# tjqansthd/GDN-Pytorch

Hardware: AMD Instinct MI355X
Metric: training images/sec at 128x416 batch=20 (higher is better)
Workload: dtype f32; 1 GPU; DtoD training step (fwd + losses + bwd + fused Adam), batch 20 per GPU, 128x416, fp32, BASELINE configs[1]; global_batch=20, parallelism=dp1, launch=eager, x3=True

## Files before the change

gdn-pytorch_amd/csrc/gemm_x3.hip:

```cpp
#include "gemm_x3.h"


namespace {

__global__ __launch_bounds__(256) void x3_pack_rows_kernel(const float* __restrict__ src, unsigned char* __restrict__ dst, int rows,
                                                           int K, int rows_pad) {
    const int KB = K / X3_BK, k8n = K / 8;
    const int bin = blockIdx.y;
    const size_t per_bin = x3_packed_bytes(rows, K);
    for (int64_t i = blockIdx.x * 256ll + threadIdx.x; i < (int64_t)rows_pad * k8n; i += (int64_t)gridDim.x * 256) {
        const int row = (int)((i >> 2) % rows_pad), k8 = (int)(i & 3) + 4 * (int)((i >> 2) / rows_pad);
        f32x4 lo = {0.f, 0.f, 0.f, 0.f}, hi = lo;
        if (row < rows) {
            const float* s = src + ((size_t)bin * rows + row) * K + k8 * 8;
            lo = *reinterpret_cast<const f32x4*>(s);
            hi = *reinterpret_cast<const f32x4*>(s + 4);
        }
        unsigned h[3][4];
        x3_split2(lo[0], lo[1], h[0][0], h[1][0], h[2][0]);
        x3_split2(lo[2], lo[3], h[0][1], h[1][1], h[2][1]);
        x3_split2(hi[0], hi[1], h[0][2], h[1][2], h[2][2]);
        x3_split2(hi[2], hi[3], h[0][3], h[1][3], h[2][3]);
#pragma unroll
        for (int p = 0; p < 3; ++p) {
            const uint4 v = {h[p][0], h[p][1], h[p][2], h[p][3]};
            *reinterpret_cast<uint4*>(dst + (size_t)bin * per_bin + x3_off(row, k8 * 8, p, KB)) = v;
        }
    }
}

__device__ __forceinline__ void x3_stage_mfma(const unsigned char* As, const unsigned char* Bs, int a_base, int b_base, int h, int f_sw,
                                              f32x16 (&acc)[2][2], f32x16 (&cor)[2][2]) {
#pragma unroll
    for (int s = 0; s < 2; ++s) {
        const int co = ((2 * s + h) ^ f_sw) * 16;
        x3_bf16x8 af[2][3], bf[2][3];
#pragma unroll
        for (int i = 0; i < 2; ++i)
#pragma unroll
            for (int p = 0; p < 3; ++p) {
                af[i][p] = __builtin_bit_cast(x3_bf16x8, *reinterpret_cast<const uint4*>(&As[p * 8192 + a_base + i * 2048 + co]));
                bf[i][p] = __builtin_bit_cast(x3_bf16x8, *reinterpret_cast<const uint4*>(&Bs[p * 8192 + b_base + i * 2048 + co]));
            }
#pragma unroll
        for (int i = 0; i < 2; ++i)
#pragma unroll
            for (int j = 0; j < 2; ++j) {
                cor[i][j] = __builtin_amdgcn_mfma_f32_32x32x16_bf16(af[i][2], bf[j][0], cor[i][j], 0, 0, 0);
                cor[i][j] = __builtin_amdgcn_mfma_f32_32x32x16_bf16(af[i][1], bf[j][1], cor[i][j], 0, 0, 0);
                cor[i][j] = __builtin_amdgcn_mfma_f32_32x32x16_bf16(af[i][0], bf[j][2], cor[i][j], 0, 0, 0);
                cor[i][j] = __builtin_amdgcn_mfma_f32_32x32x16_bf16(af[i][1], bf[j][0], cor[i][j], 0, 0, 0);
                cor[i][j] = __builtin_amdgcn_mfma_f32_32x32x16_bf16(af[i][0], bf[j][1], cor[i][j], 0, 0, 0);
                acc[i][j] = __builtin_amdgcn_mfma_f32_32x32x16_bf16(af[i][0], bf[j][0], acc[i][j], 0, 0, 0);
            }
    }
}

__global__ __launch_bounds__(256, 2) void gemm_x3_nt_kernel(const float* __restrict__ A, const unsigned char* __restrict__ Bp,
                                                            float* __restrict__ C, int M, int N, int K, int bins) {
    __shared__ __attribute__((aligned(16))) unsigned char As[3 * 128 * 64], Bs[3 * 128 * 64];
    const int tid = threadIdx.x, lane = tid & 63, wave = tid >> 6, wm = wave >> 1, wn = wave & 1;
    const int NT = N / 128, MT = (M + 127) / 128, KB = K / X3_BK;
    const int xcd = blockIdx.x & 7, sq = blockIdx.x >> 3;
    const int bin = (sq / (NT * MT)) * 8 + xcd;
    if (bin >= bins) return;
    const int m0 = ((sq / NT) % MT) * 128, nt = sq % NT;
    const float* Ab = A + (size_t)bin * M * K;
    const unsigned char* Bb = Bp + (size_t)bin * x3_packed_bytes(N, K) + (size_t)nt * KB * (3 * 128 * 64);
    float* Cb = C + (size_t)bin * M * N;

    f32x16 acc[2][2], cor[2][2];
#pragma unroll
    for (int i = 0; i < 2; ++i)
#pragma unroll
        for (int j = 0; j < 2; ++j)
#pragma unroll
            for (int r = 0; r < 16; ++r) { acc[i][j][r] = 0.f; cor[i][j][r] = 0.f; }

    const int k4 = tid & 7, rb0 = tid >> 3;
    const float* ap[4];
#pragma unroll
    for (int v = 0; v < 4; ++v) {
        const int row = v * 32 + rb0;
        ap[v] = Ab + (size_t)(m0 + row < M ? m0 + row : M - 1) * K + k4 * 4;
    }
    f32x4 ra[4];
    f32x4 rb[6];
    auto gload = [&](int kb) {
#pragma unroll
        for (int v = 0; v < 4; ++v) ra[v] = *reinterpret_cast<const f32x4*>(ap[v] + (size_t)kb * X3_BK);
        const unsigned char* bsrc = Bb + (size_t)kb * (3 * 128 * 64) + tid * 16;
#pragma unroll
        for (int v = 0; v < 6; ++v) rb[v] = *reinterpret_cast<const f32x4*>(bsrc + v * 4096);
    };
    auto lstore = [&]() {
#pragma unroll
        for (int v = 0; v < 4; ++v) {
            const int row = v * 32 + rb0;
            unsigned h0[3], h1[3];
            x3_split2(ra[v][0], ra[v][1], h0[0], h0[1], h0[2]);
            x3_split2(ra[v][2], ra[v][3], h1[0], h1[1], h1[2]);
            const int off = row * 64 + (((k4 >> 1) ^ x3_sw(row)) * 16) + (k4 & 1) * 8;
#pragma unroll
            for (int p = 0; p < 3; ++p) {
                const uint2 w = {h0[p], h1[p]};
                *reinterpret_cast<uint2*>(&As[p * 8192 + off]) = w;
            }
        }
#pragma unroll
        for (int v = 0; v < 6; ++v) *reinterpret_cast<f32x4*>(&Bs[v * 4096 + tid * 16]) = rb[v];
    };
    const int r32 = lane & 31, h = lane >> 5;
    const int f_sw = x3_sw(r32);
    const int a_base = (wm * 64 + r32) * 64, b_base = (wn * 64 + r32) * 64;

    gload(0);
    for (int kb = 0; kb < KB; ++kb) {
        lstore();
        __syncthreads();
        if (kb + 1 < KB) gload(kb + 1);
        x3_stage_mfma(As, Bs, a_base, b_base, h, f_sw, acc, cor);
        __syncthreads();
    }
#pragma unroll
    for (int i = 0; i < 2; ++i)
#pragma unroll
        for (int j = 0; j < 2; ++j) {
            const int col = nt * 128 + wn * 64 + j * 32 + r32;
#pragma unroll
            for (int r = 0; r < 16; ++r) {
                const int m = m0 + wm * 64 + i * 32 + (r & 3) + 8 * (r >> 2) + 4 * h;
                if (m < M) Cb[(size_t)m * N + col] = acc[i][j][r] + cor[i][j][r];
            }
        }
}

template <int TM>
__global__ __launch_bounds__(512, 2) void gemm_x3_nt8_kernel(const float* __restrict__ A, const unsigned char* __restrict__ Bp,
                                                             float* __restrict__ C, int M, int N, int K, int bins) {
    constexpr int MI = TM / 64, A_BYTES = 3 * TM * 64, B_BYTES = 3 * 128 * 64;
    __shared__ __attribute__((aligned(16))) unsigned char As[2][A_BYTES], Bs[2][B_BYTES];
    const int tid = threadIdx.x, lane = tid & 63, wave = tid >> 6, wm = wave >> 2, wn = wave & 3;
    const int NT = N / 128, MT = (M + TM - 1) / TM, KB = K / X3_BK;
    const int xcd = blockIdx.x & 7, sq = blockIdx.x >> 3;
    const int bin = (sq / (NT * MT)) * 8 + xcd;
    if (bin >= bins) return;
    const int m0 = ((sq / NT) % MT) * TM, nt = sq % NT;
    const float* Ab = A + (size_t)bin * M * K;
    const unsigned char* Bb = Bp + (size_t)bin * x3_packed_bytes(N, K) + (size_t)nt * KB * B_BYTES;
    float* Cb = C + (size_t)bin * M * N;
    f32x16 acc[MI], cor[MI];
#pragma unroll
    for (int i = 0; i < MI; ++i)
#pragma unroll
        for (int r = 0; r < 16; ++r) { acc[i][r] = 0.f; cor[i][r] = 0.f; }
    const int k4 = tid & 7, rb0 = tid >> 3;
    const float* ap[MI];
#pragma unroll
    for (int v = 0; v < MI; ++v) {
        const int row = v * 64 + rb0;
        ap[v] = Ab + (size_t)(m0 + row < M ? m0 + row : M - 1) * K + k4 * 4;
    }
    f32x4 ra[MI], rb[3];
    auto gload = [&](int kb) {
#pragma unroll
        for (int v = 0; v < MI; ++v) ra[v] = *reinterpret_cast<const f32x4*>(ap[v] + (size_t)kb * X3_BK);
        const unsigned char* bsrc = Bb + (size_t)kb * B_BYTES + tid * 16;
#pragma unroll
        for (int v = 0; v < 3; ++v) rb[v] = *reinterpret_cast<const f32x4*>(bsrc + v * 8192);
    };
    auto lstore = [&](int buf) {
#pragma unroll
        for (int v = 0; v < MI; ++v) {
            const int row = v * 64 + rb0;
            unsigned h0[3], h1[3];
            x3_split2(ra[v][0], ra[v][1], h0[0], h0[1], h0[2]);
            x3_split2(ra[v][2], ra[v][3], h1[0], h1[1], h1[2]);
            const int off = row * 64 + (((k4 >> 1) ^ x3_sw(row)) * 16) + (k4 & 1) * 8;
#pragma unroll
            for (int p = 0; p < 3; ++p) {
                const uint2 w = {h0[p], h1[p]};
                *reinterpret_cast<uint2*>(&As[buf][p * TM * 64 + off]) = w;
            }
        }
#pragma unroll
        for (int v = 0; v < 3; ++v) *reinterpret_cast<f32x4*>(&Bs[buf][v * 8192 + tid * 16]) = rb[v];
    };
    const int r32 = lane & 31, h = lane >> 5;
    const int f_sw = x3_sw(r32);
    const int a_base = (wm * (TM / 2) + r32) * 64, b_base = (wn * 32 + r32) * 64;
    gload(0);
    lstore(0);
    if (KB > 1) gload(1);
    __syncthreads();
    for (int kb = 0; kb < KB; ++kb) {
        const int cur = kb & 1;
        if (kb + 1 < KB) lstore(cur ^ 1);
        if (kb + 2 < KB) gload(kb + 2);
#pragma unroll
        for (int s = 0; s < 2; ++s) {
            const int co = ((2 * s + h) ^ f_sw) * 16;
            x3_bf16x8 af[MI][3], bf[3];
#pragma unroll
            for (int p = 0; p < 3; ++p) {
                bf[p] = __builtin_bit_cast(x3_bf16x8, *reinterpret_cast<const uint4*>(&Bs[cur][p * 8192 + b_base + co]));
#pragma unroll
                for (int i = 0; i < MI; ++i)
                    af[i][p] = __builtin_bit_cast(x3_bf16x8, *reinterpret_cast<const uint4*>(&As[cur][p * TM * 64 + a_base + i * 2048 + co]));
            }
#pragma unroll
            for (int i = 0; i < MI; ++i) {
                cor[i] = __builtin_amdgcn_mfma_f32_32x32x16_bf16(af[i][2], bf[0], cor[i], 0, 0, 0);
                cor[i] = __builtin_amdgcn_mfma_f32_32x32x16_bf16(af[i][1], bf[1], cor[i], 0, 0, 0);
                cor[i] = __builtin_amdgcn_mfma_f32_32x32x16_bf16(af[i][0], bf[2], cor[i], 0, 0, 0);
                cor[i] = __builtin_amdgcn_mfma_f32_32x32x16_bf16(af[i][1], bf[0], cor[i], 0, 0, 0);
                cor[i] = __builtin_amdgcn_mfma_f32_32x32x16_bf16(af[i][0], bf[1], cor[i], 0, 0, 0);
                acc[i] = __builtin_amdgcn_mfma_f32_32x32x16_bf16(af[i][0], bf[0], acc[i], 0, 0, 0);
            }
        }
        __syncthreads();
    }
    const int col = nt * 128 + wn * 32 + r32;
#pragma unroll
    for (int i = 0; i < MI; ++i)
#pragma unroll
        for (int r = 0; r < 16; ++r) {
            const int m = m0 + wm * (TM / 2) + i * 32 + (r & 3) + 8 * (r >> 2) + 4 * h;
            if (m < M) Cb[(size_t)m * N + col] = acc[i][r] + cor[i][r];
        }
}

__global__ __launch_bounds__(256, 2) void gemm_x3_tn_kernel(const float* __restrict__ A, const float* __restrict__ Bm,
                                                            float* __restrict__ P, int T, int NI, int NJ, int nsplit, int bins) {
    __shared__ __attribute__((aligned(16))) unsigned char As[3 * 128 * 64], Bs[3 * 128 * 64];
    const int tid = threadIdx.x, lane = tid & 63, wave = tid >> 6, wm = wave >> 1, wn = wave & 1;
    const int TI = NI / 128, TJ = NJ / 128;
    const int xcd = blockIdx.x & 7, sq = blockIdx.x >> 3;
    const int bin = (sq / (TI * TJ * nsplit)) * 8 + xcd;
    if (bin >= bins) return;
    const int split = (sq / (TI * TJ)) % nsplit, i0 = ((sq / TJ) % TI) * 128, j0 = (sq % TJ) * 128;
    const int chunk = ((T + nsplit - 1) / nsplit + 31) / 32 * 32;
    const int tb = split * chunk, te = tb + chunk < T ? tb + chunk : T;
    f32x16 acc[2][2], cor[2][2];
#pragma unroll
    for (int i = 0; i < 2; ++i)
#pragma unroll
        for (int j = 0; j < 2; ++j)
#pragma unroll
            for (int r = 0; r < 16; ++r) { acc[i][j][r] = 0.f; cor[i][j][r] = 0.f; }
    const int t8 = tid >> 6, cp = tid & 63;
    const float* ap = A + ((size_t)bin * T) * NI + i0 + cp;
    const float* bp = Bm + ((size_t)bin * T) * NJ + j0 + cp;
    float ra[2][8], rb[2][8];
    auto gload = [&](int t0) {
#pragma unroll
        for (int e = 0; e < 8; ++e) {
            const int t = t0 + t8 * 8 + e;
            const bool in = t < te;
            const int tc = t < T ? t : T - 1;
            const size_t ta = (size_t)tc * NI, tbo = (size_t)tc * NJ;
#pragma unroll
            for (int c = 0; c < 2; ++c) {
                const float va = ap[ta + c * 64], vb = bp[tbo + c * 64];
                ra[c][e] = in ? va : 0.f;
                rb[c][e] = in ? vb : 0.f;
            }
        }
    };
    auto lstore = [&]() {
#pragma unroll
        for (int c = 0; c < 2; ++c) {
            const int row = cp + c * 64;
            const int off = row * 64 + ((t8 ^ x3_sw(row)) * 16);
            unsigned ha[3][4], hb[3][4];
#pragma unroll
            for (int q = 0; q < 4; ++q) {
                x3_split2(ra[c][2 * q], ra[c][2 * q + 1], ha[0][q], ha[1][q], ha[2][q]);
                x3_split2(rb[c][2 * q], rb[c][2 * q + 1], hb[0][q], hb[1][q], hb[2][q]);
            }
#pragma unroll
            for (int p = 0; p < 3; ++p) {
                const uint4 va = {ha[p][0], ha[p][1], ha[p][2], ha[p][3]}, vb = {hb[p][0], hb[p][1], hb[p][2], hb[p][3]};
                *reinterpret_cast<uint4*>(&As[p * 8192 + off]) = va;
                *reinterpret_cast<uint4*>(&Bs[p * 8192 + off]) = vb;
            }
        }
    };
    const int r32 = lane & 31, h = lane >> 5;
    const int f_sw = x3_sw(r32);
    const int a_base = (wm * 64 + r32) * 64, b_base = (wn * 64 + r32) * 64;
    gload(tb);
    for (int t0 = tb; t0 < te; t0 += 32) {
        lstore();
        __syncthreads();
        if (t0 + 32 < te) gload(t0 + 32);
        x3_stage_mfma(As, Bs, a_base, b_base, h, f_sw, acc, cor);
        __syncthreads();
    }
    float* Pb = P + (((size_t)split * bins + bin) * NI) * NJ;
#pragma unroll
    for (int i = 0; i < 2; ++i)
#pragma unroll
        for (int j = 0; j < 2; ++j) {
            const int col = j0 + wn * 64 + j * 32 + r32;
#pragma unroll
            for (int r = 0; r < 16; ++r) {
                const int row = i0 + wm * 64 + i * 32 + (r & 3) + 8 * (r >> 2) + 4 * h;
                Pb[(size_t)row * NJ + col] = acc[i][j][r] + cor[i][j][r];
            }
        }
}

}

void launch_x3_pack_rows(const float* src, void* dst, int bins, int rows, int K, hipStream_t st) {
    const int rows_pad = (rows + X3_TILE - 1) / X3_TILE * X3_TILE;
    const int64_t n = (int64_t)rows_pad * (K / 8);
    const int64_t nb = cdiv64(n, 256);
    hipLaunchKernelGGL(x3_pack_rows_kernel, dim3((unsigned)(nb < 4096 ? nb : 4096), bins), dim3(256), 0, st, src,
                       (unsigned char*)dst, rows, K, rows_pad);
}

void launch_gemm_x3_nt(const float* A, const void* Bp, float* C, int bins, int M, int N, int K, hipStream_t st) {
    const int NT = N / 128, MT = (M + 127) / 128, bg = (bins + 7) / 8;
    const bool small = (int64_t)MT * NT * bins < 4 * 256;
    if (small)
        hipLaunchKernelGGL(gemm_x3_nt8_kernel<64>, dim3(((M + 63) / 64) * NT * bg * 8), dim3(512), 0, st, A, (const unsigned char*)Bp, C, M,
                           N, K, bins);
    else
        hipLaunchKernelGGL(gemm_x3_nt_kernel, dim3(MT * NT * bg * 8), dim3(256), 0, st, A, (const unsigned char*)Bp, C, M, N, K, bins);
}

void launch_gemm_x3_tn(const float* A, const float* Bm, float* P, int bins, int T, int NI, int NJ, int nsplit, hipStream_t st) {
    const int bg = (bins + 7) / 8;
    hipLaunchKernelGGL(gemm_x3_tn_kernel, dim3((NI / 128) * (NJ / 128) * nsplit * bg * 8), dim3(256), 0, st, A, Bm, P, T, NI, NJ,
                       nsplit, bins);
}

extern "C" size_t gdn_gemm_x3_packed_bytes(int32_t bins, int32_t rows, int32_t K) {
    if (bins < 1 || rows < 1 || K < X3_BK || (K % X3_BK)) return 0;
    return (size_t)bins * x3_packed_bytes(rows, K);
}

extern "C" int gdn_gemm_x3_pack(const float* src, void* dst, int32_t bins, int32_t rows, int32_t K, void* stream) {
    (void)hipGetLastError();
    if (!src || !dst || bins < 1 || rows < 1 || K < X3_BK || (K % X3_BK)) return GDN_ERR_BAD_ARG;
    launch_x3_pack_rows(src, dst, bins, rows, K, (hipStream_t)stream);
    return gdn_launch_status();
}

extern "C" int gdn_gemm_x3_nt(const float* A, const void* Bp, float* C, int32_t bins, int32_t M, int32_t N, int32_t K,
                              void* stream) {
    (void)hipGetLastError();
    if (!A || !Bp || !C || bins < 1) return GDN_ERR_BAD_ARG;
    if (!gemm_x3_ok(M, N, K)) return GDN_ERR_UNSUPPORTED;
    launch_gemm_x3_nt(A, Bp, C, bins, M, N, K, (hipStream_t)stream);
    return gdn_launch_status();
}

extern "C" int64_t gdn_gemm_x3_tn_splits(int32_t bins, int32_t T, int32_t NI, int32_t NJ) {
    if (bins < 1 || !gemm_x3_tn_ok(T, NI, NJ)) return 0;
    return gemm_x3_tn_splits(bins, T, NI, NJ);
}

extern "C" int gdn_gemm_x3_tn(const float* A, const float* Bm, float* P, int32_t bins, int32_t T, int32_t NI, int32_t NJ,
                              int32_t nsplit, void* stream) {
    (void)hipGetLastError();
    if (!A || !Bm || !P || bins < 1 || T < 1 || nsplit < 1) return GDN_ERR_BAD_ARG;
    if (!gemm_x3_tn_ok(T, NI, NJ)) return GDN_ERR_UNSUPPORTED;
    launch_gemm_x3_tn(A, Bm, P, bins, T, NI, NJ, nsplit, (hipStream_t)stream);
    return gdn_launch_status();
}
```

Measured before the change: 543.3 images/s.

## Rewrite x3 NT GEMM as persistent stream-K-style kernel with LDS DMA pipeline

Replaces the two NT GEMM variants with one persistent kernel launched with one block per CU. Each block walks a contiguous range of 32-row work groups across bins and N tiles, clipping each unit to at most eight groups. A and B tiles are double-buffered, and B is loaded straight into LDS with buffer_load ... lds, overlapped with the MFMA stages. The aim is to cut tail and launch imbalance and hide global-load latency. In exchange it adds inline asm with hand-set waitcnt counts and a cursor-based schedule that is sensitive to correctness, and it can leave waves idle on partial units.

```diff
diff --git a/gdn-pytorch_amd/csrc/gemm_x3.hip b/gdn-pytorch_amd/csrc/gemm_x3.hip
--- a/gdn-pytorch_amd/csrc/gemm_x3.hip
+++ b/gdn-pytorch_amd/csrc/gemm_x3.hip
@@ -1,4 +1,5 @@
 #include "gemm_x3.h"
+#include <type_traits>
 
 
 namespace {
@@ -56,18 +57,79 @@
     }
 }
 
-__global__ __launch_bounds__(256, 2) void gemm_x3_nt_kernel(const float* __restrict__ A, const unsigned char* __restrict__ Bp,
-                                                            float* __restrict__ C, int M, int N, int K, int bins) {
-    __shared__ __attribute__((aligned(16))) unsigned char As[3 * 128 * 64], Bs[3 * 128 * 64];
-    const int tid = threadIdx.x, lane = tid & 63, wave = tid >> 6, wm = wave >> 1, wn = wave & 1;
-    const int NT = N / 128, MT = (M + 127) / 128, KB = K / X3_BK;
-    const int xcd = blockIdx.x & 7, sq = blockIdx.x >> 3;
-    const int bin = (sq / (NT * MT)) * 8 + xcd;
-    if (bin >= bins) return;
-    const int m0 = ((sq / NT) % MT) * 128, nt = sq % NT;
-    const float* Ab = A + (size_t)bin * M * K;
-    const unsigned char* Bb = Bp + (size_t)bin * x3_packed_bytes(N, K) + (size_t)nt * KB * (3 * 128 * 64);
-    float* Cb = C + (size_t)bin * M * N;
+#define X3P_BM 256
+#define X3P_A_BYTES (3 * X3P_BM * 64)
+#define X3P_B_BYTES (3 * 128 * 64)
+#define X3P_STAGE (X3P_A_BYTES + X3P_B_BYTES)
+
+typedef __attribute__((address_space(3))) unsigned char x3_lds_u8;
+typedef int x3_i32x4 __attribute__((ext_vector_type(4)));
+
+struct X3Cursor {
+    int gi, bin, nt, gr, g, kb;
+};
+
+template <int MI, class Mid>
+__device__ __forceinline__ void x3p_stage(const unsigned char* As, const unsigned char* Bs, int a_base, int b_base, int h, int f_sw,
+                                          f32x16 (&acc)[2][2], f32x16 (&cor)[2][2], Mid&& mid) {
+#pragma unroll
+    for (int s = 0; s < 2; ++s) {
+        const int co = ((2 * s + h) ^ f_sw) * 16;
+        x3_bf16x8 af[MI][3], bf[2][3];
+#pragma unroll
+        for (int p = 0; p < 3; ++p) {
+#pragma unroll
+            for (int i = 0; i < MI; ++i)
+                af[i][p] = __builtin_bit_cast(x3_bf16x8, *reinterpret_cast<const uint4*>(&As[p * (X3P_BM * 64) + a_base + i * 8192 + co]));
+#pragma unroll
+            for (int j = 0; j < 2; ++j)
+                bf[j][p] = __builtin_bit_cast(x3_bf16x8, *reinterpret_cast<const uint4*>(&Bs[p * 8192 + b_base + j * 2048 + co]));
+        }
+        mid(s);
+#pragma unroll
+        for (int i = 0; i < MI; ++i)
+#pragma unroll
+            for (int j = 0; j < 2; ++j) {
+                cor[i][j] = __builtin_amdgcn_mfma_f32_32x32x16_bf16(af[i][2], bf[j][0], cor[i][j], 0, 0, 0);
+                cor[i][j] = __builtin_amdgcn_mfma_f32_32x32x16_bf16(af[i][1], bf[j][1], cor[i][j], 0, 0, 0);
+                cor[i][j] = __builtin_amdgcn_mfma_f32_32x32x16_bf16(af[i][0], bf[j][2], cor[i][j], 0, 0, 0);
+                cor[i][j] = __builtin_amdgcn_mfma_f32_32x32x16_bf16(af[i][1], bf[j][0], cor[i][j], 0, 0, 0);
+                cor[i][j] = __builtin_amdgcn_mfma_f32_32x32x16_bf16(af[i][0], bf[j][1], cor[i][j], 0, 0, 0);
+                acc[i][j] = __builtin_amdgcn_mfma_f32_32x32x16_bf16(af[i][0], bf[j][0], acc[i][j], 0, 0, 0);
+            }
+        __builtin_amdgcn_sched_barrier(0);
+    }
+}
+
+__global__ __launch_bounds__(512, 2) void gemm_x3_nt_kernel(const float* __restrict__ A, const unsigned char* __restrict__ Bp,
+                                                            float* __restrict__ C, int M, int N, int K, int G) {
+    __shared__ __attribute__((aligned(16))) unsigned char sm[2 * X3P_STAGE];
+    const int tid = threadIdx.x, lane = tid & 63;
+    const int wave = __builtin_amdgcn_readfirstlane(tid >> 6), wm = wave >> 1, wn = wave & 1;
+    const int NT = N / 128, GC = (M + 31) / 32, KB = K / X3_BK;
+    const size_t per_bin = x3_packed_bytes(N, K);
+
+    const int P = (int)gridDim.x, b = (int)blockIdx.x, xcd = b & 7, q = P >> 3, rq = P & 7;
+    const int v = (xcd < rq ? xcd * (q + 1) : rq * (q + 1) + (xcd - rq) * q) + (b >> 3);
+    const int g_end = (int)((int64_t)(v + 1) * G / P);
+    X3Cursor c0;
+    c0.gi = (int)((int64_t)v * G / P);
+    if (c0.gi >= g_end) return;
+    {
+        const int col = c0.gi / GC;
+        c0.gr = c0.gi - col * GC; c0.bin = col / NT; c0.nt = col - c0.bin * NT; c0.kb = 0;
+        c0.g = min(min(8, GC - c0.gr), g_end - c0.gi);
+    }
+    auto next_unit = [&](X3Cursor& c) {
+        c.kb = 0; c.gi += c.g; c.gr += c.g;
+        if (c.gr == GC) { c.gr = 0; if (++c.nt == NT) { c.nt = 0; ++c.bin; } }
+        c.g = min(min(8, GC - c.gr), g_end - c.gi);
+    };
+    auto advance = [&](X3Cursor& c) { if (++c.kb == KB) next_unit(c); };
+    X3Cursor c1 = c0;
+    advance(c1);
+    X3Cursor c2 = c1;
+    advance(c2);
 
     f32x16 acc[2][2], cor[2][2];
 #pragma unroll
@@ -78,156 +140,108 @@
             for (int r = 0; r < 16; ++r) { acc[i][j][r] = 0.f; cor[i][j][r] = 0.f; }
 
     const int k4 = tid & 7, rb0 = tid >> 3;
-    const float* ap[4];
-#pragma unroll
-    for (int v = 0; v < 4; ++v) {
-        const int row = v * 32 + rb0;
-        ap[v] = Ab + (size_t)(m0 + row < M ? m0 + row : M - 1) * K + k4 * 4;
-    }
     f32x4 ra[4];
-    f32x4 rb[6];
-    auto gload = [&](int kb) {
-#pragma unroll
-        for (int v = 0; v < 4; ++v) ra[v] = *reinterpret_cast<const f32x4*>(ap[v] + (size_t)kb * X3_BK);
-        const unsigned char* bsrc = Bb + (size_t)kb * (3 * 128 * 64) + tid * 16;
-#pragma unroll
-        for (int v = 0; v < 6; ++v) rb[v] = *reinterpret_cast<const f32x4*>(bsrc + v * 4096);
-    };
-    auto lstore = [&]() {
-#pragma unroll
-        for (int v = 0; v < 4; ++v) {
-            const int row = v * 32 + rb0;
+    auto a_load = [&](const X3Cursor& c) {
+        const int m0 = c.gr * 32, mlast = min(m0 + 32 * c.g, M) - 1;
+        const char* Ab = reinterpret_cast<const char*>(A + (size_t)c.bin * M * K + c.kb * X3_BK);
+#pragma unroll
+        for (int u = 0; u < 4; ++u) {
+            const int row = min(m0 + u * 64 + rb0, mlast);
+            ra[u] = *reinterpret_cast<const f32x4*>(Ab + (unsigned)(row * K + k4 * 4) * 4u);
+        }
+    };
+    auto a_write = [&](int buf) {
+        unsigned char* As = sm + buf * X3P_STAGE;
+#pragma unroll
+        for (int u = 0; u < 4; ++u) {
+            const int row = u * 64 + rb0;
             unsigned h0[3], h1[3];
-            x3_split2(ra[v][0], ra[v][1], h0[0], h0[1], h0[2]);
-            x3_split2(ra[v][2], ra[v][3], h1[0], h1[1], h1[2]);
+            x3_split2(ra[u][0], ra[u][1], h0[0], h0[1], h0[2]);
+            x3_split2(ra[u][2], ra[u][3], h1[0], h1[1], h1[2]);
             const int off = row * 64 + (((k4 >> 1) ^ x3_sw(row)) * 16) + (k4 & 1) * 8;
 #pragma unroll
             for (int p = 0; p < 3; ++p) {
                 const uint2 w = {h0[p], h1[p]};
-                *reinterpret_cast<uint2*>(&As[p * 8192 + off]) = w;
-            }
-        }
-#pragma unroll
-        for (int v = 0; v < 6; ++v) *reinterpret_cast<f32x4*>(&Bs[v * 4096 + tid * 16]) = rb[v];
+                *reinterpret_cast<uint2*>(&As[p * (X3P_BM * 64) + off]) = w;
+            }
+        }
+    };
+    const unsigned sm_base = (unsigned)(size_t)(x3_lds_u8*)sm, lane16 = (unsigned)lane * 16u;
+    auto b_dma = [&](const X3Cursor& c, int buf) {
+        const unsigned long long a = reinterpret_cast<unsigned long long>(Bp + (size_t)c.bin * per_bin + (size_t)c.nt * KB * X3P_B_BYTES);
+        const x3_i32x4 rs = {__builtin_amdgcn_readfirstlane((int)(unsigned)a), __builtin_amdgcn_readfirstlane((int)((unsigned)(a >> 32) & 0xffffu)),
+                             __builtin_amdgcn_readfirstlane(KB * X3P_B_BYTES), 0x00020000};
+#pragma unroll
+        for (int e = 0; e < 3; ++e) {
+            const int piece = e * 8 + wave;
+            const unsigned so = (unsigned)(c.kb * X3P_B_BYTES + piece * 1024);
+            const unsigned m0v = sm_base + (unsigned)(buf * X3P_STAGE + X3P_A_BYTES + piece * 1024);
+            asm volatile("s_mov_b32 m0, %0\n\ts_nop 0\n\tbuffer_load_dwordx4 %1, %2, %3 offen lds" :: "s"(__builtin_amdgcn_readfirstlane((int)m0v)),
+                         "v"(lane16), "s"(rs), "s"(__builtin_amdgcn_readfirstlane((int)so)) : "memory");
+        }
     };
     const int r32 = lane & 31, h = lane >> 5;
     const int f_sw = x3_sw(r32);
-    const int a_base = (wm * 64 + r32) * 64, b_base = (wn * 64 + r32) * 64;
-
-    gload(0);
-    for (int kb = 0; kb < KB; ++kb) {
-        lstore();
-        __syncthreads();
-        if (kb + 1 < KB) gload(kb + 1);
-        x3_stage_mfma(As, Bs, a_base, b_base, h, f_sw, acc, cor);
-        __syncthreads();
-    }
-#pragma unroll
-    for (int i = 0; i < 2; ++i)
-#pragma unroll
-        for (int j = 0; j < 2; ++j) {
-            const int col = nt * 128 + wn * 64 + j * 32 + r32;
-#pragma unroll
-            for (int r = 0; r < 16; ++r) {
-                const int m = m0 + wm * 64 + i * 32 + (r & 3) + 8 * (r >> 2) + 4 * h;
-                if (m < M) Cb[(size_t)m * N + col] = acc[i][j][r] + cor[i][j][r];
-            }
-        }
-}
-
-template <int TM>
-__global__ __launch_bounds__(512, 2) void gemm_x3_nt8_kernel(const float* __restrict__ A, const unsigned char* __restrict__ Bp,
-                                                             float* __restrict__ C, int M, int N, int K, int bins) {
-    constexpr int MI = TM / 64, A_BYTES = 3 * TM * 64, B_BYTES = 3 * 128 * 64;
-    __shared__ __attribute__((aligned(16))) unsigned char As[2][A_BYTES], Bs[2][B_BYTES];
-    const int tid = threadIdx.x, lane = tid & 63, wave = tid >> 6, wm = wave >> 2, wn = wave & 3;
-    const int NT = N / 128, MT = (M + TM - 1) / TM, KB = K / X3_BK;
-    const int xcd = blockIdx.x & 7, sq = blockIdx.x >> 3;
-    const int bin = (sq / (NT * MT)) * 8 + xcd;
-    if (bin >= bins) return;
-    const int m0 = ((sq / NT) % MT) * TM, nt = sq % NT;
-    const float* Ab = A + (size_t)bin * M * K;
-    const unsigned char* Bb = Bp + (size_t)bin * x3_packed_bytes(N, K) + (size_t)nt * KB * B_BYTES;
-    float* Cb = C + (size_t)bin * M * N;
-    f32x16 acc[MI], cor[MI];
-#pragma unroll
-    for (int i = 0; i < MI; ++i)
-#pragma unroll
-        for (int r = 0; r < 16; ++r) { acc[i][r] = 0.f; cor[i][r] = 0.f; }
-    const int k4 = tid & 7, rb0 = tid >> 3;
-    const float* ap[MI];
-#pragma unroll
-    for (int v = 0; v < MI; ++v) {
-        const int row = v * 64 + rb0;
-        ap[v] = Ab + (size_t)(m0 + row < M ? m0 + row : M - 1) * K + k4 * 4;
-    }
-    f32x4 ra[MI], rb[3];
-    auto gload = [&](int kb) {
-#pragma unroll
-        for (int v = 0; v < MI; ++v) ra[v] = *reinterpret_cast<const f32x4*>(ap[v] + (size_t)kb * X3_BK);
-        const unsigned char* bsrc = Bb + (size_t)kb * B_BYTES + tid * 16;
-#pragma unroll
-        for (int v = 0; v < 3; ++v) rb[v] = *reinterpret_cast<const f32x4*>(bsrc + v * 8192);
-    };
-    auto lstore = [&](int buf) {
-#pragma unroll
-        for (int v = 0; v < MI; ++v) {
-            const int row = v * 64 + rb0;
-            unsigned h0[3], h1[3];
-            x3_split2(ra[v][0], ra[v][1], h0[0], h0[1], h0[2]);
-            x3_split2(ra[v][2], ra[v][3], h1[0], h1[1], h1[2]);
-            const int off = row * 64 + (((k4 >> 1) ^ x3_sw(row)) * 16) + (k4 & 1) * 8;
-#pragma unroll
-            for (int p = 0; p < 3; ++p) {
-                const uint2 w = {h0[p], h1[p]};
-                *reinterpret_cast<uint2*>(&As[buf][p * TM * 64 + off]) = w;
-            }
-        }
-#pragma unroll
-        for (int v = 0; v < 3; ++v) *reinterpret_cast<f32x4*>(&Bs[buf][v * 8192 + tid * 16]) = rb[v];
-    };
-    const int r32 = lane & 31, h = lane >> 5;
-    const int f_sw = x3_sw(r32);
-    const int a_base = (wm * (TM / 2) + r32) * 64, b_base = (wn * 32 + r32) * 64;
-    gload(0);
-    lstore(0);
-    if (KB > 1) gload(1);
-    __syncthreads();
-    for (int kb = 0; kb < KB; ++kb) {
-        const int cur = kb & 1;
-        if (kb + 1 < KB) lstore(cur ^ 1);
-        if (kb + 2 < KB) gload(kb + 2);
-#pragma unroll
-        for (int s = 0; s < 2; ++s) {
-            const int co = ((2 * s + h) ^ f_sw) * 16;
-            x3_bf16x8 af[MI][3], bf[3];
-#pragma unroll
-            for (int p = 0; p < 3; ++p) {
-                bf[p] = __builtin_bit_cast(x3_bf16x8, *reinterpret_cast<const uint4*>(&Bs[cur][p * 8192 + b_base + co]));
-#pragma unroll
-                for (int i = 0; i < MI; ++i)
-                    af[i][p] = __builtin_bit_cast(x3_bf16x8, *reinterpret_cast<const uint4*>(&As[cur][p * TM * 64 + a_base + i * 2048 + co]));
-            }
-#pragma unroll
-            for (int i = 0; i < MI; ++i) {
-                cor[i] = __builtin_amdgcn_mfma_f32_32x32x16_bf16(af[i][2], bf[0], cor[i], 0, 0, 0);
-                cor[i] = __builtin_amdgcn_mfma_f32_32x32x16_bf16(af[i][1], bf[1], cor[i], 0, 0, 0);
-                cor[i] = __builtin_amdgcn_mfma_f32_32x32x16_bf16(af[i][0], bf[2], cor[i], 0, 0, 0);
-                cor[i] = __builtin_amdgcn_mfma_f32_32x32x16_bf16(af[i][1], bf[0], cor[i], 0, 0, 0);
-                cor[i] = __builtin_amdgcn_mfma_f32_32x32x16_bf16(af[i][0], bf[1], cor[i], 0, 0, 0);
-                acc[i] = __builtin_amdgcn_mfma_f32_32x32x16_bf16(af[i][0], bf[0], acc[i], 0, 0, 0);
-            }
-        }
-        __syncthreads();
-    }
-    const int col = nt * 128 + wn * 32 + r32;
-#pragma unroll
-    for (int i = 0; i < MI; ++i)
-#pragma unroll
-        for (int r = 0; r < 16; ++r) {
-            const int m = m0 + wm * (TM / 2) + i * 32 + (r & 3) + 8 * (r >> 2) + 4 * h;
-            if (m < M) Cb[(size_t)m * N + col] = acc[i][r] + cor[i][r];
-        }
+    const int a_base = (wm * 32 + r32) * 64, b_base = (wn * 64 + r32) * 64;
+
+    a_load(c0);
+    a_write(0);
+    b_dma(c0, 0);
+    a_load(c1.gi < g_end ? c1 : c0);
+    asm volatile("s_waitcnt vmcnt(4) lgkmcnt(0)" ::: "memory");
+    __builtin_amdgcn_s_barrier();
+    asm volatile("" ::: "memory");
+    int buf = 0;
+    auto run_unit = [&](auto mi) {
+        constexpr int MI = decltype(mi)::value;
+        for (int kb = 0; kb < KB; ++kb) {
+            auto mid = [&](int sub) {
+                if (sub == 0) {
+                    a_write(buf ^ 1);
+                } else {
+                    b_dma(c1.gi < g_end ? c1 : c0, buf ^ 1);
+                    a_load(c2.gi < g_end ? c2 : c0);
+                }
+            };
+            if constexpr (MI > 0) {
+                const unsigned char* As = sm + buf * X3P_STAGE;
+                x3p_stage<MI>(As, As + X3P_A_BYTES, a_base, b_base, h, f_sw, acc, cor, mid);
+            } else {
+                mid(0);
+                mid(1);
+            }
+            asm volatile("s_waitcnt vmcnt(4) lgkmcnt(0)" ::: "memory");
+            __builtin_amdgcn_s_barrier();
+            asm volatile("" ::: "memory");
+            buf ^= 1;
+            c1 = c2;
+            advance(c2);
+        }
+    };
+    for (;;) {
+        const int g = c0.g;
+        if (wm + 4 < g) run_unit(std::integral_constant<int, 2>{});
+        else if (wm < g) run_unit(std::integral_constant<int, 1>{});
+        else run_unit(std::integral_constant<int, 0>{});
+        const int m0 = c0.gr * 32, mend = min(m0 + 32 * g, M);
+        float* Cb = C + (size_t)c0.bin * M * N;
+#pragma unroll
+        for (int i = 0; i < 2; ++i)
+#pragma unroll
+            for (int j = 0; j < 2; ++j) {
+                const int col = c0.nt * 128 + wn * 64 + j * 32 + r32;
+#pragma unroll
+                for (int r = 0; r < 16; ++r) {
+                    const int m = m0 + (wm + 4 * i) * 32 + (r & 3) + 8 * (r >> 2) + 4 * h;
+                    if (m < mend) Cb[(size_t)m * N + col] = acc[i][j][r] + cor[i][j][r];
+                    acc[i][j][r] = 0.f;
+                    cor[i][j][r] = 0.f;
+                }
+            }
+        next_unit(c0);
+        if (c0.gi >= g_end) break;
+    }
+    asm volatile("s_waitcnt vmcnt(0)" ::: "memory");
 }
 
 __global__ __launch_bounds__(256, 2) void gemm_x3_tn_kernel(const float* __restrict__ A, const float* __restrict__ Bm,
@@ -322,13 +336,9 @@
 }
 
 void launch_gemm_x3_nt(const float* A, const void* Bp, float* C, int bins, int M, int N, int K, hipStream_t st) {
-    const int NT = N / 128, MT = (M + 127) / 128, bg = (bins + 7) / 8;
-    const bool small = (int64_t)MT * NT * bins < 4 * 256;
-    if (small)
-        hipLaunchKernelGGL(gemm_x3_nt8_kernel<64>, dim3(((M + 63) / 64) * NT * bg * 8), dim3(512), 0, st, A, (const unsigned char*)Bp, C, M,
-                           N, K, bins);
-    else
-        hipLaunchKernelGGL(gemm_x3_nt_kernel, dim3(MT * NT * bg * 8), dim3(256), 0, st, A, (const unsigned char*)Bp, C, M, N, K, bins);
+    const int64_t G = (int64_t)bins * (N / 128) * ((M + 31) / 32);
+    const int P = (int)(G < gdn_num_cus() ? G : gdn_num_cus());
+    hipLaunchKernelGGL(gemm_x3_nt_kernel, dim3(P), dim3(512), 0, st, A, (const unsigned char*)Bp, C, M, N, K, (int)G);
 }
 
 void launch_gemm_x3_tn(const float* A, const float* Bm, float* P, int bins, int T, int NI, int NJ, int nsplit, hipStream_t st) {
```

Measured after the change: 546.1 images/s (median of 6 runs). No clear change (+0.5%).
